# dazchi/gym-uav-collision-avoidance

Hardware: NVIDIA B200
Metric: UAV env-steps/sec (higher is better)
Workload: dtype f64 velocity / f32 position+obs (as the reference)

## Files before the change

gym_uav_collision_avoidance_b200/csrc/uavca_kernels.cu:

```cuda
#include <atomic>
#include <cmath>
#include <cstdlib>

#include "uavca_host.h"
#include "uavca_multi.cuh"
#include "uavca_seq.cuh"
#include "uavca_cta.cuh"
#include "uavca_tma.cuh"

namespace uavca {


struct GlobalIO {
  const KernelArgs& a;
  const Lane& L;
  float* stage;
  __device__ __forceinline__ Uav load_uav() const { return uavca::load_uav(a.s, L); }
  __device__ __forceinline__ float2 load_action() const {
    return L.valid ? ld_stream(a.io.action + L.m) : make_float2(0.f, 0.f);
  }
  __device__ __forceinline__ int load_steps() const { return L.valid ? a.s.steps[L.env] : 0; }
  __device__ __forceinline__ void loads_done() const { cudaTriggerProgrammaticLaunchCompletion(); }
  __device__ __forceinline__ void store_reward_done(float r, bool done) const {
    if (L.valid) {
// ... 279 lines not shown
                      L.valid ? a.s.steps[L.env] : 0, (unsigned)L.m};
    cudaTriggerProgrammaticLaunchCompletion();
    const unsigned M = (unsigned)r.M;
    if constexpr (KIND == kRolloutPlainBlock) {
      const unsigned end = r.KM + (unsigned)L.m;
      if (L.valid) cp_async8(slot, r.action_block + io.off);
      do {
        cp_async_wait_all();
        io.act = L.valid ? lds_float2(slot) : make_float2(0.f, 0.f);
        const unsigned next = io.off + M;
        if (next < end && L.valid) cp_async8(slot ^ 256u, r.action_block + next);
        step_core<NT>(a, ws, L, io);
        io.off = next;
        slot ^= 256u;
      } while (io.off < end);
    } else {
      uint4 words = make_uint4(0u, 0u, 0u, 0u);
      for (int k = 0; k < r.K; ++k) {
        const unsigned long long t = r.step0 + (unsigned long long)k;
        if (k == 0 || (t & 1ull) == 0ull) words = action_words(r.seed_lo, r.seed_hi, env_global, L.i, t);
        io.act = map_action(action_from_words(words, t), UAVCA_ACTION_SCALED, a.c);
        step_core<NT>(a, ws, L, io);
        io.off += M;
      }
    }
    store_uav(a.s, L, io.cur, true);
    if (L.valid & (L.i == 0)) a.s.steps[L.env] = io.steps;
  } else {
    const bool block = r.action_block != nullptr;
    RolloutIO io{a, r, L, ws.stage, load_uav(a.s, L), make_float2(0.f, 0.f), L.valid ? a.s.steps[L.env] : 0, 0, 0};
    cudaTriggerProgrammaticLaunchCompletion();
    if (block && L.valid) cp_async8(slot, r.action_block + L.m);
    uint4 words = make_uint4(0u, 0u, 0u, 0u);
    for (int k = 0; k < r.K; ++k) {
      io.k = k;
      io.km = (long long)k * r.M;
      if (block) {
        cp_async_wait_all();
        io.act = L.valid ? lds_float2(slot + (k & 1) * 256) : make_float2(0.f, 0.f);
        if (k + 1 < r.K && L.valid) cp_async8(slot + ((k + 1) & 1) * 256, (r.action_block + (io.km + r.M)) + (unsigned)L.m);
      } else {
        const unsigned long long t = r.step0 + (unsigned long long)k;
        if (k == 0 || (t & 1ull) == 0ull) words = action_words(r.seed_lo, r.seed_hi, env_global, L.i, t);
        io.act = action_from_words(words, t);
        if (r.action_out != nullptr && L.valid) st_stream((r.action_out + io.km) + L.m, io.act);
      }
      step_core<NT>(a, ws, L, io);
    }
    store_uav(a.s, L, io.cur, true);
    if (L.valid & (L.i == 0)) a.s.steps[L.env] = io.steps;
  }
}

#ifndef UAVCA_ROLLOUT_MINB
#define UAVCA_ROLLOUT_MINB 8
#endif
template <int NT, int KIND>
__global__ void __launch_bounds__(kThreads, UAVCA_ROLLOUT_MINB) rollout_multi_kernel(const __grid_constant__ KernelArgs a,
                                                                                  const __grid_constant__ RolloutArgs r) {
  __shared__ __align__(16) float smem[kWarpsPerBlock * kScratchFloats];
  __shared__ __align__(512) float2 act_smem[kWarpsPerBlock * 64];
  const WarpScratch ws = warp_scratch(smem);
  const int warp_global = blockIdx.x * kWarpsPerBlock + (threadIdx.x >> 5);
  const int N = NT > 0 ? NT : a.N;
  const bool full = uavs_left(a.B, N, warp_global) >= (32 / N) * N;
  cudaGridDependencySynchronize();
  float2* const my_act = act_smem + (threadIdx.x >> 5) * 64;
  if (full) rollout_multi_body<NT, true, KIND>(a, r, ws, my_act, warp_global);
  else rollout_multi_body<NT, false, KIND>(a, r, ws, my_act, warp_global);
}

__global__ void __launch_bounds__(kThreads) sample_actions_kernel(const __grid_constant__ Consts c, float2* out, int B, int N,
                                                                  unsigned seed_lo, unsigned seed_hi, unsigned long long t) {
  const long long m = (long long)blockIdx.x * kThreads + threadIdx.x;
  if (m >= (long long)B * N) return;
  const long long env = m / N;
  const int i = (int)(m - env * N);
  out[m] = action_from_words(action_words(seed_lo, seed_hi, c.env_base + env, i, t), t);
}

constexpr int kPfStageBytes = 32 * (16 + 8 + 8 + 8 + 4 + 4);


struct PfStage {
  double2* vel;
  float2 *pos, *tgt, *act;
  float *init, *prev;
};
__device__ __forceinline__ PfStage pf_stage(unsigned char* base) {
  PfStage st;
  st.vel = reinterpret_cast<double2*>(base);
  st.pos = reinterpret_cast<float2*>(base + 32 * 16);
  st.tgt = st.pos + 32;
  st.act = st.tgt + 32;
  st.init = reinterpret_cast<float*>(st.act + 32);
  st.prev = st.init + 32;
  return st;
}

struct PfIO : GlobalIO {
  Uav pre;
  float2 act;
  int steps;
  __device__ __forceinline__ Uav load_uav() const { return pre; }
  __device__ __forceinline__ float2 load_action() const { return act; }
  __device__ __forceinline__ int load_steps() const { return steps; }
// ... 370 lines not shown
                                                                 float* o_mask, long long* o_idx) {
  const long long j = ((long long)blockIdx.x * kThreads + threadIdx.x) / kSampleLanes;
  const int l = threadIdx.x % kSampleLanes;
  if (j >= batch) return;
  const long long head = meta[0], size = meta[2];
  const unsigned long long ctr = draw + (unsigned long long)meta[3];
  const uint4 r = philox_indexed(kStreamSample, (unsigned long long)j, ctr, seed_lo, seed_hi);
  long long slot = 0;
  if (size > 0) {
    if (recency) {
      const double u = ((double)r.x + 0.5) * (1.0 / 4294967296.0);
      long long age = (long long)(sqrt(u) * (double)size);
      age = age >= size ? size - 1 : age;
      const long long oldest = size == cap ? head : 0;
      slot = oldest + age;
      slot -= slot >= cap ? cap : 0;
    } else {
      slot = (long long)(((unsigned long long)r.x * (unsigned long long)size) >> 32);
    }
  }
  for (int k = l; k < od; k += kSampleLanes) {
    o_obs[j * od + k] = r_obs[slot * od + k];
    o_nxt[j * od + k] = r_nxt[slot * od + k];
  }
  for (int k = l; k < ad; k += kSampleLanes) o_act[j * ad + k] = r_act[slot * ad + k];
  if (l == 0) {
    o_rew[j] = r_rew[slot];
    o_mask[j] = r_mask[slot];
    if (o_idx) o_idx[j] = slot;
  }
}


static inline int flat_grid(long long n) { return (int)((n + kThreads - 1) / kThreads); }

static inline int multi_grid(int B, int N) {
  const int epw = 32 / N;
  const long long warps = ((long long)B + epw - 1) / epw;
  return (int)((warps + kWarpsPerBlock - 1) / kWarpsPerBlock);
}

#define UAVCA_DISPATCH_N(N, CALL)            \
  switch (N) {                               \
    case 2: { constexpr int NT = 2; CALL; } break;   \
    case 4: { constexpr int NT = 4; CALL; } break;   \
    case 5: { constexpr int NT = 5; CALL; } break;   \
    case 8: { constexpr int NT = 8; CALL; } break;   \
    case 10: { constexpr int NT = 10; CALL; } break; \
    case 16: { constexpr int NT = 16; CALL; } break; \
    case 32: { constexpr int NT = 32; CALL; } break; \
    default: { constexpr int NT = 0; CALL; } break;  \
  }

template <int NT>
static cudaError_t launch_step_multi_n(const KernelArgs& a, int grid, cudaStream_t st) {
  cudaLaunchConfig_t cfg{};
  cfg.gridDim = dim3(grid);
  cfg.blockDim = dim3(kThreads);
  cfg.dynamicSmemBytes = 0;
  cfg.stream = st;
  cudaLaunchAttribute attr[1];
  attr[0].id = cudaLaunchAttributeProgrammaticStreamSerialization;
  attr[0].val.programmaticStreamSerializationAllowed = 1;
  cfg.attrs = attr;
  cfg.numAttrs = 1;
  return cudaLaunchKernelEx(&cfg, step_multi_kernel<NT>, a);
}


template <typename Kernel>
static cudaError_t launch_pdl(Kernel kernel, int grid, int threads, size_t smem, cudaStream_t st, const KernelArgs& a,
                              int num_tiles) {
  cudaLaunchConfig_t cfg{};
  cfg.gridDim = dim3(grid);
  cfg.blockDim = dim3(threads);
  cfg.dynamicSmemBytes = smem;
  cfg.stream = st;
  cudaLaunchAttribute attr[1];
  attr[0].id = cudaLaunchAttributeProgrammaticStreamSerialization;
  attr[0].val.programmaticStreamSerializationAllowed = 1;
  cfg.attrs = attr;
  cfg.numAttrs = 1;
  return cudaLaunchKernelEx(&cfg, kernel, a, num_tiles);
}

template <int NT, bool FINAL>
static cudaError_t launch_step_tma_n(const KernelArgs& a, int num_tiles, cudaStream_t st) {
  using G = TmaGeom<NT, FINAL>;
  constexpr int kMaxDev = 64;
  static std::atomic<int> slots[kMaxDev];
  int dev = 0;
  cudaError_t e = cudaGetDevice(&dev);
  if (e != cudaSuccess) return e;
  if (dev < 0 || dev >= kMaxDev) return cudaErrorInvalidDevice;
  auto kernel = step_multi_tma_kernel<NT, FINAL>;
  if (slots[dev] == 0) {
    e = cudaFuncSetAttribute(kernel, cudaFuncAttributeMaxDynamicSharedMemorySize, G::SMEM_BYTES);
    if (e != cudaSuccess) return e;
    int per_sm = 0, sms = 0;
    e = cudaOccupancyMaxActiveBlocksPerMultiprocessor(&per_sm, kernel, G::THREADS, G::SMEM_BYTES);
    if (e != cudaSuccess) return e;
    e = cudaDeviceGetAttribute(&sms, cudaDevAttrMultiProcessorCount, dev);
    if (e != cudaSuccess) return e;
    if (per_sm < 1) return cudaErrorLaunchOutOfResources;
    slots[dev] = per_sm * sms;
  }
// ... 173 lines not shown
  cfg.gridDim = dim3(grid);
  cfg.blockDim = dim3(kThreads);
  cfg.dynamicSmemBytes = 0;
  cfg.stream = st;
  cudaLaunchAttribute attr[1];
  attr[0].id = cudaLaunchAttributeProgrammaticStreamSerialization;
  attr[0].val.programmaticStreamSerializationAllowed = 1;
  cfg.attrs = attr;
  cfg.numAttrs = 1;
  return cudaLaunchKernelEx(&cfg, step_multi_ring_kernel<NT>, a, g);
}

cudaError_t launch_step_multi_ring(const KernelArgs& a, const RingSink& g, cudaStream_t st) {
  if (a.B <= 0) return cudaSuccess;
  if (wants_seq(a)) return cudaErrorNotSupported;
  cudaError_t e = cudaSuccess;
  UAVCA_DISPATCH_N(a.N, (e = launch_step_multi_ring_n<NT>(a, g, multi_grid(a.B, a.N), st)));
  if (e != cudaSuccess) return e;
  return cudaGetLastError();
}

template <typename Kernel>
static cudaError_t launch_pdl2(Kernel kernel, int grid, cudaStream_t st, const KernelArgs& a, const RolloutArgs& r) {
  cudaLaunchConfig_t cfg{};
  cfg.gridDim = dim3(grid);
  cfg.blockDim = dim3(kThreads);
  cfg.dynamicSmemBytes = 0;
  cfg.stream = st;
  cudaLaunchAttribute attr[1];
  attr[0].id = cudaLaunchAttributeProgrammaticStreamSerialization;
  attr[0].val.programmaticStreamSerializationAllowed = 1;
  cfg.attrs = attr;
  cfg.numAttrs = 1;
  return cudaLaunchKernelEx(&cfg, kernel, a, r);
}

cudaError_t launch_rollout_multi(const KernelArgs& a, const RolloutArgs& r, cudaStream_t st) {
  if (a.B <= 0 || r.K <= 0) return cudaSuccess;
  cudaError_t e = cudaSuccess;
  static const bool cta_ok = [] { const char* v = getenv("UAVCA_ROLLOUT_CTA"); return !(v && v[0] == '0'); }();
  if (cta_ok && cta_packs(a.N, true)) {
    const int envs_per_cta = kThreads / a.N;
    e = launch_pdl2(rollout_multi_cta_kernel, (a.B + envs_per_cta - 1) / envs_per_cta, st, a, r);
    return e != cudaSuccess ? e : cudaGetLastError();
  }
  const int grid = multi_grid(a.B, a.N);
  const bool block = r.action_block != nullptr;
  const bool plain = a.io.final_obs == nullptr && a.io.reset_mask == nullptr && !a.c.track_scores &&
                     (block ? a.io.action_mode == UAVCA_ACTION_CARTESIAN
                            : a.io.action_mode == UAVCA_ACTION_SCALED && r.action_out == nullptr) &&
                     (long long)r.K * r.M * UAVCA_OBS_DIM_MULTI < (1ll << 31);
  RolloutArgs rp = r;
  rp.KM = plain ? (unsigned)(r.K * r.M) : 0u;
  if (block && plain) {
    UAVCA_DISPATCH_N(a.N, (e = launch_pdl2(rollout_multi_kernel<NT, kRolloutPlainBlock>, grid, st, a, rp)));
  } else if (plain) {
    UAVCA_DISPATCH_N(a.N, (e = launch_pdl2(rollout_multi_kernel<NT, kRolloutPlainPhilox>, grid, st, a, rp)));
  } else {
    UAVCA_DISPATCH_N(a.N, (e = launch_pdl2(rollout_multi_kernel<NT, kRolloutGeneral>, grid, st, a, r)));
  }
  return e != cudaSuccess ? e : cudaGetLastError();
}

cudaError_t launch_rollout_single(const KernelArgs& a, const RolloutArgs& r, cudaStream_t st) {
  if (a.B <= 0 || r.K <= 0) return cudaSuccess;
  const cudaError_t e = launch_pdl2(rollout_single_kernel, flat_grid(a.B), st, a, r);
  return e != cudaSuccess ? e : cudaGetLastError();
}

cudaError_t launch_sample_actions(const Consts& c, float* out, int B, int N, unsigned long long seed, unsigned long long t,
                                  cudaStream_t st) {
  if (B <= 0) return cudaSuccess;
  sample_actions_kernel<<<flat_grid((long long)B * N), kThreads, 0, st>>>(c, reinterpret_cast<float2*>(out), B, N,
                                                                          (unsigned)(seed & 0xffffffffull),
                                                                          (unsigned)(seed >> 32), t);
  return cudaGetLastError();
}

cudaError_t launch_reset_multi(const KernelArgs& a, const uint8_t* mask, cudaStream_t st) {
  if (a.B <= 0) return cudaSuccess;
  if (wants_seq(a)) {
    if (a.c.circular) reset_multi_seq_kernel<double><<<flat_grid(a.B), kThreads, 0, st>>>(a, mask);
    else reset_multi_seq_kernel<float><<<flat_grid(a.B), kThreads, 0, st>>>(a, mask);
    return cudaGetLastError();
  }
  const int grid = multi_grid(a.B, a.N);
  UAVCA_DISPATCH_N(a.N, (reset_multi_kernel<NT><<<grid, kThreads, 0, st>>>(a, mask)));
  return cudaGetLastError();
}

cudaError_t launch_observe_multi(const KernelArgs& a, cudaStream_t st) {
  if (a.B <= 0) return cudaSuccess;
  if (wants_seq(a)) {
    if (a.c.circular) observe_multi_seq_kernel<double><<<flat_grid(a.B), kThreads, 0, st>>>(a);
    else observe_multi_seq_kernel<float><<<flat_grid(a.B), kThreads, 0, st>>>(a);
    return cudaGetLastError();
  }
  const int grid = multi_grid(a.B, a.N);
  UAVCA_DISPATCH_N(a.N, (observe_multi_kernel<NT><<<grid, kThreads, 0, st>>>(a)));
  return cudaGetLastError();
}

cudaError_t launch_step_single(const KernelArgs& a, cudaStream_t st) {
  if (a.B <= 0) return cudaSuccess;
  step_single_kernel<<<flat_grid(a.B), kThreads, 0, st>>>(a);
  return cudaGetLastError();
// ... 67 lines not shown
```

gym_uav_collision_avoidance_b200/csrc/uavca_multi.cuh:

```cuda
#pragma once

#include "uavca_device.cuh"

namespace uavca {

struct Lane {
  int N;
  int lanes_used;
  int lane;
  int i;
  int base;
  int ring;
  unsigned envmask;
  int env;
  int m;
  int warp_m0;
  int valid_lanes;
  bool valid;
};

__device__ __forceinline__ int uavs_left(int B, int N, int warp_global) { return (B - warp_global * (32 / N)) * N; }

template <int NT, bool FULL = false>
__device__ __forceinline__ Lane make_lane(int B, int Nrt, int warp_global) {
// ... 25 lines not shown
  return make_lane<NT, false>(B, Nrt, blockIdx.x * kWarpsPerBlock + (threadIdx.x >> 5));
}

struct Uav {
  float px, py, tx, ty, init, prev;
  double vx, vy;
  unsigned flags;
};

__device__ __forceinline__ Uav load_uav(const StateView& s, const Lane& L) {
  Uav u;
  if (L.valid) {
    float2 p = ld_stream(s.pos + L.m);
    double2 v = ld_stream(s.vel + L.m);
    float2 t = ld_stream(s.tgt + L.m);
    u.init = ld_stream(s.init + L.m);
    u.prev = ld_stream(s.prev + L.m);
    u.flags = ld_stream(s.flags + L.m);
    u.px = p.x; u.py = p.y; u.vx = v.x; u.vy = v.y; u.tx = t.x; u.ty = t.y;
  } else {
    u.px = u.py = u.ty = 0.f; u.tx = 8.f; u.init = u.prev = 8.f; u.vx = 1.0; u.vy = 0.0; u.flags = 0u;
  }
  return u;
}

__device__ __forceinline__ void store_uav(const StateView& s, const Lane& L, const Uav& u, bool with_target) {
  if (!L.valid) return;
  st_stream(s.pos + L.m, make_float2(u.px, u.py));
  st_stream(s.vel + L.m, make_double2(u.vx, u.vy));
  st_stream(s.prev + L.m, u.prev);
  st_stream(s.flags + L.m, (uint8_t)u.flags);
  if (with_target) {
    st_stream(s.tgt + L.m, make_float2(u.tx, u.ty));
    st_stream(s.init + L.m, u.init);
  }
}

struct WarpScratch {
  float4* pairs;
  float4* cand;
  float* th;
  float* stage;
  __device__ __forceinline__ float4* ring() const { return pairs; }
  __device__ __forceinline__ float* ring_th() const { return reinterpret_cast<float*>(pairs) + 256; }
};
constexpr int kMixedMaxN = 10;
template <int NT>
struct SweepKind {
  static constexpr bool kMixed = NT > 0 && NT <= kMixedMaxN;
};
constexpr int kRingFloats = 48 * 4 + 32 * 4 + 32;
constexpr int kScratchFloats = kRingFloats + 32 * 10;

__device__ __forceinline__ WarpScratch warp_scratch(float* block_smem) {
  float* w = block_smem + (threadIdx.x >> 5) * kScratchFloats;
  return WarpScratch{reinterpret_cast<float4*>(w), reinterpret_cast<float4*>(w + 192), w + 320, w + kRingFloats};
}

__device__ __forceinline__ void publish(const WarpScratch& ws, const Lane& L, float nx, float ny, float ox, float oy, float th_u) {
  if (L.valid) {
    float* ring = reinterpret_cast<float*>(ws.pairs + L.ring);
    const int s0 = L.i, s1 = L.i + L.N;
    const int a0 = ((s0 >> 1) << 2) + (s0 & 1), a1 = ((s1 >> 1) << 2) + (s1 & 1);
    ring[a0] = nx; ring[a0 + 2] = ny;
    ring[a1] = nx; ring[a1 + 2] = ny;
    ws.cand[L.lane] = make_float4(nx, ny, ox, oy);
    ws.th[L.lane] = th_u;
  }
  __syncwarp();
}


constexpr int kInfBits = 0x7f800000;

static __device__ __noinline__ int nearest2_exact(const float4* cand, int i, int N, float px, float py) {
  const float inf = __int_as_float(kInfBits);
  float s1 = inf, s2 = inf;
  int j1 = 0, j2 = 0;
  for (int k = 1; k < N; ++k) {
    int j = i + k;
    j -= j >= N ? N : 0;
    const float4 q = cand[j];
    const float s = sq32(__fsub_rn(q.x, px), __fsub_rn(q.y, py));
    const bool p1 = s < s1, p2 = s < s2;
    j2 = p1 ? j1 : (p2 ? k : j2);
    s2 = p1 ? s1 : (p2 ? s : s2);
    j1 = p1 ? k : j1;
    s1 = p1 ? s : s1;
  }
  return j1 | (j2 << 8);
}

static __device__ __noinline__ float nearest_mixed_exact(const float4* cand, int i, int N, float px, float py) {
  float smin = __int_as_float(kInfBits);
  for (int j = 0; j < N; ++j) {
    if (j == i) continue;
    const float4 q = cand[j];
    const float s = j < i ? sq32(__fsub_rn(q.x, px), __fsub_rn(q.y, py)) : sq32(__fsub_rn(q.z, px), __fsub_rn(q.w, py));
    smin = fminf(smin, s);
  }
  return smin;
}

template <int NT>
__device__ __forceinline__ void pair_scan(const Consts& c, const WarpScratch& ws, const Lane& L, float px, float py,
                                          int& k1, int& k2, int& t3_out) {
  const int N = NT > 0 ? NT : L.N;
  const int k0 = L.i & 1;
  const float4* row = ws.pairs + L.ring + ((L.i + 1) >> 1);
  const float2 npx = make_float2(-px, -px), npy = make_float2(-py, -py), zero = make_float2(0.f, 0.f);
  auto dist2 = [&](int p) {
    const float4 q = row[p];
    const float2 dx = __fadd2_rn(make_float2(q.x, q.y), npx), dy = __fadd2_rn(make_float2(q.z, q.w), npy);
    return __fadd2_rn(__ffma2_rn(dx, dx, zero), __ffma2_rn(dy, dy, zero));
  };
  const int mask = c.key_mask;
  auto key = [&](float sq, int e) {
    int kk = (__float_as_int(sq) & mask) | e;
    if (e >= N) return kInfBits + 5 * 32;
    if (e == 0) kk = k0 ? kk : kInfBits + 3 * 32;
    if (e == N - 1) kk = k0 ? kInfBits + 4 * 32 : kk;
    return kk;
// ... 35 lines not shown
  float2 a, b, c;
};
__device__ __forceinline__ ObsTail obs_tail(const Consts& c, float dx1, float dy1, float dx2, float dy2, float s1, float s2,
                                            float h1, float h2, bool have1, bool have2, float th_u) {
  const float2 b = fast_atan2_pair(dy1, dx1, dy2, dx2);
  const float2 nth = make_float2(-th_u, -th_u);
  const float2 v1 = wrap_units2(__ffma2_rn(b, make_float2(c.inv_pi, c.inv_pi), nth));
  const float2 v2 = wrap_units2(__fadd2_rn(make_float2(h1, h2), nth));
  const float2 d = __fmul2_rn(make_float2(sqrt_approx(s1), sqrt_approx(s2)), make_float2(c.inv_dsense, c.inv_dsense));
  ObsTail o;
  o.a.x = have1 ? d.x : 1.0f;
  o.a.y = have1 ? v1.x : 1.0f;
  o.b.x = have1 ? v2.x : 0.0f;
  o.b.y = have2 ? d.y : 1.0f;
  o.c.x = have2 ? v1.y : 1.0f;
  o.c.y = have2 ? v2.y : 0.0f;
  return o;
}

template <int NT, bool WANT_A>
__device__ __forceinline__ ObsTail neighbours(const Consts& c, const WarpScratch& ws, const Lane& L, float px, float py,
                                              float th_u, int k1, int k2, int t3, float& smin) {
  const int N = NT > 0 ? NT : L.N;
  int j1 = L.i + k1, j2 = L.i + k2;
  const bool w1 = j1 >= N, w2 = j2 >= N;
  j1 -= w1 ? N : 0;
  j2 -= w2 ? N : 0;
  const float4 q1 = ws.cand[L.base + j1], q2 = ws.cand[L.base + j2];
  const float h1 = ws.th[L.base + j1], h2 = ws.th[L.base + j2];
  const float dx1 = __fsub_rn(q1.x, px), dy1 = __fsub_rn(q1.y, py), dx2 = __fsub_rn(q2.x, px), dy2 = __fsub_rn(q2.y, py);
  const float s1 = sq32(dx1, dy1), s2 = sq32(dx2, dy2);
  if (WANT_A) {
    const float inf = __int_as_float(kInfBits);
    float a1 = w1 ? s1 : sq32(__fsub_rn(q1.z, px), __fsub_rn(q1.w, py));
    float a2 = w2 ? s2 : sq32(__fsub_rn(q2.z, px), __fsub_rn(q2.w, py));
    a1 = k1 != 0 ? a1 : inf;
    a2 = k2 != 0 ? a2 : inf;
    smin = fminf(a1, a2);
    if (t3 <= c.near_key) smin = nearest_mixed_exact(ws.cand + L.base, L.i, N, px, py);
  }
  const bool have1 = (k1 != 0) & (s1 < c.s_dsense_lt);
  const bool have2 = have1 & (k2 != 0) & (s2 < c.s_dsense_lt);
  return obs_tail(c, dx1, dy1, dx2, dy2, s1, s2, h1, h2, have1, have2, th_u);
}

__device__ __forceinline__ void publish_mixed(const WarpScratch& ws, const Lane& L, float nx, float ny, float ox, float oy, float th_u) {
  if (L.valid) {
    const int slot = 2 * L.base + L.i;
    ws.ring()[slot] = make_float4(ox, nx, oy, ny);
    ws.ring()[slot + L.N] = make_float4(nx, nx, ny, ny);
    ws.ring_th()[slot] = th_u;
    ws.ring_th()[slot + L.N] = th_u;
  }
  __syncwarp();
}

static __device__ __noinline__ int nearest2_exact_ring(const float4* row, float px, float py, int N) {
  const float inf = __int_as_float(kInfBits);
  float s1 = inf, s2 = inf;
  int j1 = 0, j2 = 0;
  for (int k = 1; k < N; ++k) {
    const float4 q = row[k];
    const float s = sq32(__fsub_rn(q.y, px), __fsub_rn(q.w, py));
    const bool p1 = s < s1, p2 = s < s2;
    j2 = p1 ? j1 : (p2 ? k : j2);
    s2 = p1 ? s1 : (p2 ? s : s2);
    j1 = p1 ? k : j1;
    s1 = p1 ? s : s1;
  }
  return j1 | (j2 << 8);
}

template <int NT>
__device__ __forceinline__ void pair_scan_mixed(const Consts& c, const WarpScratch& ws, const Lane& L, float px, float py,
                                                float& smin, int& k1, int& k2) {
  constexpr int N = NT;
  const float4* row = ws.ring() + 2 * L.base + L.i;
  const float2 npx = make_float2(-px, -px), npy = make_float2(-py, -py), zero = make_float2(0.f, 0.f);
  auto dist2 = [&](int k) {
    const float4 q = row[k];
    const float2 dx = __fadd2_rn(make_float2(q.x, q.y), npx), dy = __fadd2_rn(make_float2(q.z, q.w), npy);
    return __fadd2_rn(__ffma2_rn(dx, dx, zero), __ffma2_rn(dy, dy, zero));
  };
  const int mask = c.key_mask;
  auto key = [mask](float sq, int k) { return (__float_as_int(sq) & mask) | k; };
  smin = __int_as_float(kInfBits);
  int t1 = kInfBits, t2 = kInfBits + 32, t3 = kInfBits + 64;
  int k = 1;
#pragma unroll
  for (; k + 1 < N; k += 2) {
    const float2 s0 = dist2(k), s1 = dist2(k + 1);
    smin = fminf(smin, fminf(s0.x, s1.x));
    const int ka = key(s0.y, k), kb = key(s1.y, k + 1);
    const int a = min(ka, kb), b = max(ka, kb);
    const int m1a = max(t1, a), m2a = max(t2, a), m1b = max(t1, b);
    t3 = __vimin3_s32(t3, m2a, m1b);
    t2 = __vimin3_s32(t2, m1a, b);
    t1 = min(t1, a);
  }
  if (k < N) {
    const float2 s0 = dist2(k);
    smin = fminf(smin, s0.x);
    const int a = key(s0.y, k);
    t3 = min(t3, max(t2, a));
    t2 = min(t2, max(t1, a));
    t1 = min(t1, a);
  }
  k1 = t1 & 31;
  k2 = t2 & 31;
  if (((unsigned)(t1 ^ t2) < 32u) | ((unsigned)(t2 ^ t3) < 32u)) {
    const int e = nearest2_exact_ring(row, px, py, N);
    k1 = e & 0xff;
    k2 = e >> 8;
  }
}

__device__ __forceinline__ ObsTail neighbours_mixed(const Consts& c, const WarpScratch& ws, const Lane& L, float px, float py,
                                                    float th_u, int k1, int k2) {
  const int slot = 2 * L.base + L.i;
  const float4 q1 = ws.ring()[slot + k1], q2 = ws.ring()[slot + k2];
  const float h1 = ws.ring_th()[slot + k1], h2 = ws.ring_th()[slot + k2];
  const float2 dx = __fadd2_rn(make_float2(q1.y, q2.y), make_float2(-px, -px)), dy = __fadd2_rn(make_float2(q1.w, q2.w), make_float2(-py, -py));
  const float2 zero = make_float2(0.f, 0.f), s = __fadd2_rn(__ffma2_rn(dx, dx, zero), __ffma2_rn(dy, dy, zero));
  const bool have1 = (k1 != 0) & (s.x < c.s_dsense_lt);
  const bool have2 = have1 & (k2 != 0) & (s.y < c.s_dsense_lt);
  return obs_tail(c, dx.x, dy.x, dx.y, dy.y, s.x, s.y, h1, h2, have1, have2, th_u);
}

template <int NT>
__device__ __forceinline__ ObsTail scan_neighbours(const Consts& c, const WarpScratch& ws, const Lane& L, float nx, float ny,
                                                   float ox, float oy, float th_u, float& smin) {
  int k1, k2;
  if (SweepKind<NT>::kMixed) {
    publish_mixed(ws, L, nx, ny, ox, oy, th_u);
    pair_scan_mixed<NT>(c, ws, L, nx, ny, smin, k1, k2);
    return neighbours_mixed(c, ws, L, nx, ny, th_u, k1, k2);
  }
  int t3;
  publish(ws, L, nx, ny, ox, oy, th_u);
  pair_scan<NT>(c, ws, L, nx, ny, k1, k2, t3);
  return neighbours<NT, true>(c, ws, L, nx, ny, th_u, k1, k2, t3, smin);
}

struct Own {
  float th_u, dth_u, dist, ssq;
  double vsq;
};
__device__ __forceinline__ Own own_features(const Consts& c, float px, float py, float tx, float ty, double vx, double vy) {
  Own w;
  const float2 td = __fadd2_rn(make_float2(tx, ty), make_float2(-px, -py));
  const float tdx = td.x, tdy = td.y;
  const float2 tsq = __ffma2_rn(td, td, make_float2(0.f, 0.f));
  w.ssq = __fadd_rn(tsq.x, tsq.y);
  w.dist = __fsqrt_rn(w.ssq);
  w.vsq = sq64(vx, vy);
  const float fvx = (float)vx, fvy = (float)vy;
  const bool vzero = (vx == 0.0) & (vy == 0.0);
  const float hx = vzero ? 1.0f : fvx;
  const float cr = fmaf(hx, tdy, -(fvy * tdx));
  const float dt = fmaf(hx, tdx, fvy * tdy);
  const float2 ang = fast_atan2_pair(fvy, fvx, cr, dt);
  w.th_u = ang.x * c.inv_pi;
  w.dth_u = ang.y * c.inv_pi;
  if ((!vzero & (fabsf(fvx) + fabsf(fvy) < 1e-30f)) | (w.ssq == 0.0f)) {
    const float2 s = angles_slow((double)tdx, (double)tdy, vx, vy);
    w.th_u = s.x; w.dth_u = s.y;
  }
  return w;
}

__device__ __forceinline__ void obs_own(const Consts& c, const Own& w, double vsq, float2& o01, float2& o23) {
  o01 = make_float2(sqrt_approx((float)vsq) * c.inv_vm2_f, w.th_u);
  o23 = make_float2(w.dist * c.inv_diag, w.dth_u);
}

struct ObsRow {
  float2 o01, o23;
  ObsTail n;
};
template <int NT>
__device__ __forceinline__ ObsRow observe_state(const Consts& c, const WarpScratch& ws, const Lane& L, const Uav& u) {
  const Own w = own_features(c, u.px, u.py, u.tx, u.ty, u.vx, u.vy);
  __syncwarp();
  ObsRow r;
  obs_own(c, w, w.vsq, r.o01, r.o23);
  float unused;
  r.n = scan_neighbours<NT>(c, ws, L, u.px, u.py, u.px, u.py, w.th_u, unused);
  return r;
}

__device__ __forceinline__ void stage_own(float* stage, int lane, float2 o01, float2 o23) {
  float2* row = reinterpret_cast<float2*>(stage) + lane * 5;
  row[0] = o01; row[1] = o23;
}
// ... 130 lines not shown
    const bool env_conflict = ((bal >> L.base) & L.envmask) != 0u;
    if (active) {
      if (env_conflict && att + 1u < kMaxResetAttempts) {
        if (L.i == cur) {
          ++attempt;
          tg = draw_pair(c, env_global, episode, kStreamTgt, L.i, attempt, c.lox, c.hix, c.loy, c.hiy);
        }
      } else {
        ++cur;
      }
    }
  }
  if (do_reset) {
    u.px = cand.x; u.py = cand.y; u.tx = tg.x; u.ty = tg.y;
    u.vx = 0.0; u.vy = 0.0; u.flags = 0u;
    u.init = n32(__fsub_rn(u.tx, u.px), __fsub_rn(u.ty, u.py));
    u.prev = u.init;
  }
}


__device__ __forceinline__ float env_sum(float v, const Lane& L) {
#pragma unroll
  for (int off = 1; off < 32; off <<= 1) {
    const float o = __shfl_down_sync(kFull, v, off);
    v += (L.i + off < L.N) ? o : 0.0f;
  }
  return v;
}

__device__ __forceinline__ void fold_scores(const StateView& s, int env) {
  const double2 sc = s.score[env];
  atomicAdd(reinterpret_cast<double*>(s.stats + 4), sc.x);
  atomicAdd(reinterpret_cast<double*>(s.stats + 5), sc.y);
  s.score[env] = make_double2(0.0, 0.0);
}

static __device__ __forceinline__ double2 finish_velocity(double vx, double vy, double vsq) {
  const double nv = sqrt(vsq);
  double fx = __dmul_rn(__ddiv_rn(vx, nv), 0.001), fy = __dmul_rn(__ddiv_rn(vy, nv), 0.001);
  if ((fx != fx) | (fy != fy)) { fx = 0.0; fy = 0.0; }
  return make_double2(fx, fy);
}

template <class IO, class = void>
struct io_action64 { static constexpr bool value = false; };
template <class IO>
struct io_action64<IO, decltype((void)IO::kAction64)> { static constexpr bool value = IO::kAction64; };
template <class IO, class = void>
struct io_plain { static constexpr bool value = false; };
template <class IO>
struct io_plain<IO, decltype((void)IO::kPlain)> { static constexpr bool value = IO::kPlain; };

template <int NT, class IO>
__device__ __forceinline__ void step_core(const KernelArgs& a, const WarpScratch& ws, const Lane& L, IO& io) {
  const Consts& c = a.c;
  constexpr bool kF64 = io_action64<IO>::value;
  constexpr bool kPlain = io_plain<IO>::value;

  Uav u = io.load_uav();
  float2 act = make_float2(0.f, 0.f);
  double2 act64 = make_double2(0.0, 0.0);
  if constexpr (kF64) act64 = io.load_action64();
  else act = io.load_action();
  const int steps_new = io.load_steps() + 1;
  io.loads_done();
  if constexpr (!kF64 && !kPlain) {
    if (a.io.action_mode != UAVCA_ACTION_CARTESIAN) act = map_action(act, a.io.action_mode, c);
  }

  const bool parked = (u.flags & UAVCA_FLAG_PARKED) != 0u;
  const float ox = u.px, oy = u.py;

  {
    double vx = u.vx, vy = u.vy;
    float px = u.px, py = u.py;
    if constexpr (kF64) integrate(act64.x, act64.y, vx, vy, px, py, c);
    else integrate((double)act.x, (double)act.y, vx, vy, px, py, c);
    if (!parked) { u.vx = vx; u.vy = vy; u.px = px; u.py = py; }
  }
  const Own w = own_features(c, u.px, u.py, u.tx, u.ty, u.vx, u.vy);
  const float dist = parked ? 0.f : w.dist;
  const float prev_d = parked ? 0.f : u.prev;

  float r;
  {
    const float inv_init = rcp_approx(u.init);
    const float m = fminf(c.vm2_f * inv_init, 1.0f);
    r = fmaf(50.0f * c.inv_vm2_f, __fsub_rn(prev_d, dist), -0.01f * m);
    const float q = dist * inv_init * (1.0f / 1.5f);
    r *= (r > 0.0f) ? (1.0f - q) : (1.0f + q);
    r = fmaf(-0.01f * 3.14159274101257324f, fabsf(w.dth_u), r);
  }

  float smin;
  const ObsTail tail = scan_neighbours<NT>(c, ws, L, u.px, u.py, ox, oy, w.th_u, smin);

  const bool collision = smin <= c.s_coll_le;
  r = collision ? -2.0f : r;
  const bool hard = (smin <= c.s_hard_le) & ((u.flags & (UAVCA_FLAG_PARKED | UAVCA_FLAG_COLLIDED)) == 0u) & L.valid;
  if (hard) u.flags |= UAVCA_FLAG_COLLIDED;

  const bool inside = (u.px >= c.lox_f) & (u.px <= c.hix_f) & (u.py >= c.loy_f) & (u.py <= c.hiy_f);
  const bool reached = (parked ? true : (w.ssq < c.s_reach_lt)) & !collision & (w.vsq < c.reach_speed_sq);
  const bool newly_reached = reached & !parked & L.valid;
  const bool done = (reached | (!inside & (a.io.evaluate == 0))) & L.valid;
  double vsq_obs = w.vsq;
  if (reached) {
    u.flags |= UAVCA_FLAG_PARKED;
    const double2 fv = finish_velocity(u.vx, u.vy, w.vsq);
    u.vx = fv.x; u.vy = fv.y;
    r += 10.0f;
    vsq_obs = sq64(u.vx, u.vy);
  }
  u.prev = dist;

  {
    float2 o01, o23;
    obs_own(c, w, vsq_obs, o01, o23);
    io.put_own(o01, o23);
    io.put_neighbours(tail);
  }
  io.store_reward_done(r, done);

  const unsigned done_env = (__ballot_sync(kFull, done) >> L.base) & L.envmask;
  const bool rs = (((done_env & c.rs_any_mask) != 0u) | (((done_env ^ L.envmask) | c.rs_all_off) == 0u) |
                   (steps_new >= c.steps_limit)) & L.valid;
  const bool leader = L.valid & (L.i == 0);
  if (leader) io.store_reset(rs);
  if (!kPlain && c.track_scores) {
    const float live = env_sum((done | !L.valid) ? 0.0f : r, L);
    if (leader) {
      double2 sc = a.s.score[L.env];
      sc.x += (double)r;
      sc.y += (double)live;
      a.s.score[L.env] = sc;
    }
  }
  const bool bad = (!(fabsf(r) <= 3.4e38f) | !(fabsf(u.px) + fabsf(u.py) <= 3.4e38f)) & L.valid;

  if (!__any_sync(kFull, rs | newly_reached | hard | bad)) {
    io.store_steps(steps_new, leader);
    io.commit_obs();
    if (io.wants_final()) io.commit_final();
    io.store_state(u);
    return;
  }

  const unsigned ev_reach = __ballot_sync(kFull, newly_reached), ev_coll = __ballot_sync(kFull, hard);
  const int reach_inc = __popc((ev_reach >> L.base) & L.envmask), coll_inc = __popc((ev_coll >> L.base) & L.envmask);
  {
    const unsigned ev_bad = __ballot_sync(kFull, bad);
    if (ev_bad != 0u && L.lane == 0) atomicAdd(a.s.stats + 6, (unsigned long long)__popc(ev_bad));
  }
  if (io.wants_final()) io.commit_final();
  if (!__any_sync(kFull, rs)) {
    io.store_steps(steps_new, leader);
    if (leader) {
      if (reach_inc) a.s.reach[L.env] += reach_inc;
      if (coll_inc) a.s.coll[L.env] += coll_inc;
    }
    io.commit_obs();
    io.store_state(u);
    return;
  }
  unsigned episode = 0;
  if (leader) episode = a.s.episode[L.env];
  episode = __shfl_sync(kFull, episode, L.base);
  if (leader) {
    if (rs) {
      if (episode > 0u) {
        atomicAdd(a.s.stats + 0, 1ull);
        atomicAdd(a.s.stats + 1, (unsigned long long)(a.s.reach[L.env] + reach_inc));
        atomicAdd(a.s.stats + 2, (unsigned long long)(a.s.coll[L.env] + coll_inc));
        atomicAdd(a.s.stats + 3, (unsigned long long)steps_new);
        if (c.track_scores) fold_scores(a.s, L.env);
      }
      a.s.reach[L.env] = 0; a.s.coll[L.env] = 0;
      a.s.episode[L.env] = episode + 1u;
    } else {
      if (reach_inc) a.s.reach[L.env] += reach_inc;
      if (coll_inc) a.s.coll[L.env] += coll_inc;
    }
  }
  io.store_steps(rs ? 0 : steps_new, leader);
  Uav nu = u;
  reset_multi(a, L, rs, episode, nu);
  const ObsRow no = observe_state<NT>(c, ws, L, nu);
  if (rs) {
    u = nu;
    io.put_own(no.o01, no.o23);
    io.put_neighbours(no.n);
  }
  io.commit_obs();
  io.store_state(u);
  if (rs) io.store_target(u);
}

}
```

Before: 56.30 billion.

## Process two warps' worth of environments per warp in plain rollout

Adds a paired rollout kernel in which each warp steps two warp-groups of environments, interleaving their movement, neighbour publish, sweep and settle phases. The two groups share one warp sync and one any-vote check for the rare path, and observation rows are staged in shared memory and flushed as coalesced float4 streams. The aim is more independent work per warp to hide latency, along with amortised syncs and action prefetches. In exchange, register and shared-memory use grow (minimum blocks per SM drops to 4), which lowers occupancy, and the rare path runs serially for both groups.

```diff
diff --git a/gym_uav_collision_avoidance_b200/csrc/uavca_kernels.cu b/gym_uav_collision_avoidance_b200/csrc/uavca_kernels.cu
--- a/gym_uav_collision_avoidance_b200/csrc/uavca_kernels.cu
+++ b/gym_uav_collision_avoidance_b200/csrc/uavca_kernels.cu
@@ -355,6 +355,113 @@
   }
 }
 
+struct PairRolloutIO : PlainRolloutIO {
+  __device__ __forceinline__ void put_own(float2 o01, float2 o23) const {
+    if (L.valid) stage_own(stage, L.lane, o01, o23);
+  }
+  __device__ __forceinline__ void put_neighbours(const ObsTail& n) const {
+    if (L.valid) stage_neighbours(stage, L.lane, n);
+  }
+  __device__ __forceinline__ void commit_obs() const {}
+};
+
+template <int NT>
+__device__ __forceinline__ void flush_pair_rows(unsigned stage, float* g, int lane) {
+  constexpr int n4 = (32 / NT) * NT * 5;
+  float4* g4 = reinterpret_cast<float4*>(g);
+  __syncwarp();
+#pragma unroll
+  for (int r = 0; r < (n4 + 31) / 32; ++r) {
+    const int k = lane + 32 * r;
+    if (k < n4) st_stream(g4 + k, lds_float4(stage + k * 16));
+  }
+  __syncwarp();
+}
+
+template <int NT, int KIND>
+__device__ __forceinline__ void rollout_multi_pair_body(const KernelArgs& a, const RolloutArgs& r, const WarpScratch& wsA,
+                                                        const WarpScratch& wsB, unsigned stage, unsigned slot, int pair) {
+  constexpr int kUsed = (32 / NT) * NT;
+  const Lane LA = make_lane<NT, true>(a.B, a.N, 2 * pair), LB = make_lane<NT, true>(a.B, a.N, 2 * pair + 1);
+  const bool valid = LA.valid;
+  PairRolloutIO ioA{{a, LA, stage, load_uav(a.s, LA), make_float2(0.f, 0.f), valid ? a.s.steps[LA.env] : 0, (unsigned)LA.m}};
+  PairRolloutIO ioB{{a, LB, stage + kUsed * 40u, load_uav(a.s, LB), make_float2(0.f, 0.f), valid ? a.s.steps[LB.env] : 0,
+                     (unsigned)LB.m}};
+  cudaTriggerProgrammaticLaunchCompletion();
+  const unsigned M = (unsigned)r.M;
+  auto obs_run = [&] { return a.io.obs + (ioA.off - (unsigned)LA.lane) * (unsigned)UAVCA_OBS_DIM_MULTI; };
+  if constexpr (KIND == kRolloutPlainBlock) {
+    const unsigned end = r.KM + (unsigned)LA.m;
+    if (valid) {
+      cp_async8(slot, r.action_block + ioA.off);
+      cp_async8(slot + 512u, r.action_block + (ioA.off + kUsed));
+    }
+    do {
+      cp_async_wait_all();
+      ioA.act = valid ? lds_float2(slot) : make_float2(0.f, 0.f);
+      ioB.act = valid ? lds_float2(slot + 512u) : make_float2(0.f, 0.f);
+      const unsigned next = ioA.off + M;
+      if (next < end && valid) {
+        cp_async8(slot ^ 256u, r.action_block + next);
+        cp_async8((slot ^ 256u) + 512u, r.action_block + (next + kUsed));
+      }
+      ioB.off = ioA.off + kUsed;
+      step_pair<NT>(a, wsA, wsB, LA, LB, ioA, ioB);
+      flush_pair_rows<NT>(stage, obs_run(), LA.lane);
+      ioA.off = next;
+      slot ^= 256u;
+    } while (ioA.off < end);
+  } else {
+    const long long envA = a.c.env_base + LA.env, envB = a.c.env_base + LB.env;
+    uint4 wa = make_uint4(0u, 0u, 0u, 0u), wb = wa;
+    for (int k = 0; k < r.K; ++k) {
+      const unsigned long long t = r.step0 + (unsigned long long)k;
+      if (k == 0 || (t & 1ull) == 0ull) {
+        wa = action_words(r.seed_lo, r.seed_hi, envA, LA.i, t);
+        wb = action_words(r.seed_lo, r.seed_hi, envB, LB.i, t);
+      }
+      ioA.act = map_action(action_from_words(wa, t), UAVCA_ACTION_SCALED, a.c);
+      ioB.act = map_action(action_from_words(wb, t), UAVCA_ACTION_SCALED, a.c);
+      ioB.off = ioA.off + kUsed;
+      step_pair<NT>(a, wsA, wsB, LA, LB, ioA, ioB);
+      flush_pair_rows<NT>(stage, obs_run(), LA.lane);
+      ioA.off += M;
+    }
+  }
+  store_uav(a.s, LA, ioA.cur, true);
+  store_uav(a.s, LB, ioB.cur, true);
+  if (valid & (LA.i == 0)) {
+    a.s.steps[LA.env] = ioA.steps;
+    a.s.steps[LB.env] = ioB.steps;
+  }
+}
+
+#ifndef UAVCA_ROLLOUT_PAIR_MINB
+#define UAVCA_ROLLOUT_PAIR_MINB 4
+#endif
+constexpr int kPairWarpFloats = 2 * kRingFloats + 64 * 10;
+template <int NT, int KIND>
+__global__ void __launch_bounds__(kThreads, UAVCA_ROLLOUT_PAIR_MINB)
+    rollout_multi_pair_kernel(const __grid_constant__ KernelArgs a, const __grid_constant__ RolloutArgs r) {
+  __shared__ __align__(16) float smem[kWarpsPerBlock * kPairWarpFloats];
+  __shared__ __align__(512) float2 act_smem[kWarpsPerBlock * 128];
+  float* const w = smem + (threadIdx.x >> 5) * kPairWarpFloats;
+  float* const stage = w + 2 * kRingFloats;
+  const WarpScratch wsA = scratch_at(w, stage), wsB = scratch_at(w + kRingFloats, stage);
+  float2* const my_act = act_smem + (threadIdx.x >> 5) * 128;
+  const int pair = blockIdx.x * kWarpsPerBlock + (threadIdx.x >> 5);
+  constexpr int kUsed = (32 / NT) * NT;
+  const int left = uavs_left(a.B, NT, 2 * pair);
+  cudaGridDependencySynchronize();
+  if (left >= 2 * kUsed) {
+    rollout_multi_pair_body<NT, KIND>(a, r, wsA, wsB, (unsigned)__cvta_generic_to_shared(stage),
+                                      (unsigned)__cvta_generic_to_shared(my_act + (threadIdx.x & 31)), pair);
+  } else if (left > 0) {
+    rollout_multi_body<NT, false, KIND>(a, r, wsA, my_act, 2 * pair);
+    if (left > kUsed) rollout_multi_body<NT, false, KIND>(a, r, wsA, my_act, 2 * pair + 1);
+  }
+}
+
 #ifndef UAVCA_ROLLOUT_MINB
 #define UAVCA_ROLLOUT_MINB 8
 #endif
@@ -831,6 +938,18 @@
     default: { constexpr int NT = 0; CALL; } break;  \
   }
 
+#define UAVCA_DISPATCH_PAIR_N(N, CALL)                   \
+  switch (N) {                                           \
+    case 2: { constexpr int NT = 2; CALL; } break;       \
+    case 4: { constexpr int NT = 4; CALL; } break;       \
+    case 5: { constexpr int NT = 5; CALL; } break;       \
+    case 8: { constexpr int NT = 8; CALL; } break;       \
+    case 10: { constexpr int NT = 10; CALL; } break;     \
+    case 16: { constexpr int NT = 16; CALL; } break;     \
+    case 32: { constexpr int NT = 32; CALL; } break;     \
+    default: break;                                      \
+  }
+
 template <int NT>
 static cudaError_t launch_step_multi_n(const KernelArgs& a, int grid, cudaStream_t st) {
   cudaLaunchConfig_t cfg{};
@@ -1110,6 +1229,18 @@
                      (long long)r.K * r.M * UAVCA_OBS_DIM_MULTI < (1ll << 31);
   RolloutArgs rp = r;
   rp.KM = plain ? (unsigned)(r.K * r.M) : 0u;
+  if (plain) {
+    bool paired = false;
+    const int epw = 32 / a.N;
+    const long long pairs = (((long long)a.B + epw - 1) / epw + 1) / 2;
+    const int pgrid = (int)((pairs + kWarpsPerBlock - 1) / kWarpsPerBlock);
+    if (block) {
+      UAVCA_DISPATCH_PAIR_N(a.N, (paired = true, e = launch_pdl2(rollout_multi_pair_kernel<NT, kRolloutPlainBlock>, pgrid, st, a, rp)));
+    } else {
+      UAVCA_DISPATCH_PAIR_N(a.N, (paired = true, e = launch_pdl2(rollout_multi_pair_kernel<NT, kRolloutPlainPhilox>, pgrid, st, a, rp)));
+    }
+    if (paired) return e != cudaSuccess ? e : cudaGetLastError();
+  }
   if (block && plain) {
     UAVCA_DISPATCH_N(a.N, (e = launch_pdl2(rollout_multi_kernel<NT, kRolloutPlainBlock>, grid, st, a, rp)));
   } else if (plain) {
diff --git a/gym_uav_collision_avoidance_b200/csrc/uavca_multi.cuh b/gym_uav_collision_avoidance_b200/csrc/uavca_multi.cuh
--- a/gym_uav_collision_avoidance_b200/csrc/uavca_multi.cuh
+++ b/gym_uav_collision_avoidance_b200/csrc/uavca_multi.cuh
@@ -101,9 +101,12 @@
 constexpr int kRingFloats = 48 * 4 + 32 * 4 + 32;
 constexpr int kScratchFloats = kRingFloats + 32 * 10;
 
+__device__ __forceinline__ WarpScratch scratch_at(float* w, float* stage) {
+  return WarpScratch{reinterpret_cast<float4*>(w), reinterpret_cast<float4*>(w + 192), w + 320, stage};
+}
 __device__ __forceinline__ WarpScratch warp_scratch(float* block_smem) {
   float* w = block_smem + (threadIdx.x >> 5) * kScratchFloats;
-  return WarpScratch{reinterpret_cast<float4*>(w), reinterpret_cast<float4*>(w + 192), w + 320, w + kRingFloats};
+  return scratch_at(w, w + kRingFloats);
 }
 
 __device__ __forceinline__ void publish(const WarpScratch& ws, const Lane& L, float nx, float ny, float ox, float oy, float th_u) {
@@ -116,7 +119,6 @@
     ws.cand[L.lane] = make_float4(nx, ny, ox, oy);
     ws.th[L.lane] = th_u;
   }
-  __syncwarp();
 }
 
 
@@ -258,7 +260,6 @@
     ws.ring_th()[slot] = th_u;
     ws.ring_th()[slot + L.N] = th_u;
   }
-  __syncwarp();
 }
 
 static __device__ __noinline__ int nearest2_exact_ring(const float4* row, float px, float py, int N) {
@@ -334,18 +335,29 @@
 }
 
 template <int NT>
+__device__ __forceinline__ void publish_neighbours(const WarpScratch& ws, const Lane& L, float nx, float ny, float ox, float oy,
+                                                   float th_u) {
+  if (SweepKind<NT>::kMixed) publish_mixed(ws, L, nx, ny, ox, oy, th_u);
+  else publish(ws, L, nx, ny, ox, oy, th_u);
+}
+template <int NT>
+__device__ __forceinline__ ObsTail sweep_neighbours(const Consts& c, const WarpScratch& ws, const Lane& L, float nx, float ny,
+                                                    float th_u, float& smin) {
+  int k1, k2;
+  if (SweepKind<NT>::kMixed) {
+    pair_scan_mixed<NT>(c, ws, L, nx, ny, smin, k1, k2);
+    return neighbours_mixed(c, ws, L, nx, ny, th_u, k1, k2);
+  }
+  int t3;
+  pair_scan<NT>(c, ws, L, nx, ny, k1, k2, t3);
+  return neighbours<NT, true>(c, ws, L, nx, ny, th_u, k1, k2, t3, smin);
+}
+template <int NT>
 __device__ __forceinline__ ObsTail scan_neighbours(const Consts& c, const WarpScratch& ws, const Lane& L, float nx, float ny,
                                                    float ox, float oy, float th_u, float& smin) {
-  int k1, k2;
-  if (SweepKind<NT>::kMixed) {
-    publish_mixed(ws, L, nx, ny, ox, oy, th_u);
-    pair_scan_mixed<NT>(c, ws, L, nx, ny, smin, k1, k2);
-    return neighbours_mixed(c, ws, L, nx, ny, th_u, k1, k2);
-  }
-  int t3;
-  publish(ws, L, nx, ny, ox, oy, th_u);
-  pair_scan<NT>(c, ws, L, nx, ny, k1, k2, t3);
-  return neighbours<NT, true>(c, ws, L, nx, ny, th_u, k1, k2, t3, smin);
+  publish_neighbours<NT>(ws, L, nx, ny, ox, oy, th_u);
+  __syncwarp();
+  return sweep_neighbours<NT>(c, ws, L, nx, ny, th_u, smin);
 }
 
 struct Own {
@@ -582,25 +594,36 @@
 template <class IO>
 struct io_plain<IO, decltype((void)IO::kPlain)> { static constexpr bool value = IO::kPlain; };
 
+struct StepVals {
+  Uav u;
+  Own w;
+  float r, dist, ox, oy;
+  int steps_new;
+  bool parked, done, rs, newly_reached, hard, bad, leader;
+};
+
 template <int NT, class IO>
-__device__ __forceinline__ void step_core(const KernelArgs& a, const WarpScratch& ws, const Lane& L, IO& io) {
+__device__ __forceinline__ StepVals step_move(const KernelArgs& a, const Lane& L, IO& io) {
   const Consts& c = a.c;
   constexpr bool kF64 = io_action64<IO>::value;
   constexpr bool kPlain = io_plain<IO>::value;
-
-  Uav u = io.load_uav();
+  StepVals s;
+  Uav& u = s.u;
+
+  u = io.load_uav();
   float2 act = make_float2(0.f, 0.f);
   double2 act64 = make_double2(0.0, 0.0);
   if constexpr (kF64) act64 = io.load_action64();
   else act = io.load_action();
-  const int steps_new = io.load_steps() + 1;
+  s.steps_new = io.load_steps() + 1;
   io.loads_done();
   if constexpr (!kF64 && !kPlain) {
     if (a.io.action_mode != UAVCA_ACTION_CARTESIAN) act = map_action(act, a.io.action_mode, c);
   }
 
   const bool parked = (u.flags & UAVCA_FLAG_PARKED) != 0u;
-  const float ox = u.px, oy = u.py;
+  s.parked = parked;
+  s.ox = u.px; s.oy = u.py;
 
   {
     double vx = u.vx, vy = u.vy;
@@ -609,22 +632,31 @@
     else integrate((double)act.x, (double)act.y, vx, vy, px, py, c);
     if (!parked) { u.vx = vx; u.vy = vy; u.px = px; u.py = py; }
   }
-  const Own w = own_features(c, u.px, u.py, u.tx, u.ty, u.vx, u.vy);
-  const float dist = parked ? 0.f : w.dist;
+  s.w = own_features(c, u.px, u.py, u.tx, u.ty, u.vx, u.vy);
+  const float dist = parked ? 0.f : s.w.dist;
   const float prev_d = parked ? 0.f : u.prev;
-
-  float r;
+  s.dist = dist;
+
   {
     const float inv_init = rcp_approx(u.init);
     const float m = fminf(c.vm2_f * inv_init, 1.0f);
-    r = fmaf(50.0f * c.inv_vm2_f, __fsub_rn(prev_d, dist), -0.01f * m);
+    float r = fmaf(50.0f * c.inv_vm2_f, __fsub_rn(prev_d, dist), -0.01f * m);
     const float q = dist * inv_init * (1.0f / 1.5f);
     r *= (r > 0.0f) ? (1.0f - q) : (1.0f + q);
-    r = fmaf(-0.01f * 3.14159274101257324f, fabsf(w.dth_u), r);
-  }
-
-  float smin;
-  const ObsTail tail = scan_neighbours<NT>(c, ws, L, u.px, u.py, ox, oy, w.th_u, smin);
+    s.r = fmaf(-0.01f * 3.14159274101257324f, fabsf(s.w.dth_u), r);
+  }
+  return s;
+}
+
+template <int NT, class IO>
+__device__ __forceinline__ void step_settle(const KernelArgs& a, const Lane& L, IO& io, StepVals& s, const ObsTail& tail,
+                                            float smin) {
+  const Consts& c = a.c;
+  constexpr bool kPlain = io_plain<IO>::value;
+  Uav& u = s.u;
+  const Own& w = s.w;
+  const bool parked = s.parked;
+  float r = s.r;
 
   const bool collision = smin <= c.s_coll_le;
   r = collision ? -2.0f : r;
@@ -643,7 +675,7 @@
     r += 10.0f;
     vsq_obs = sq64(u.vx, u.vy);
   }
-  u.prev = dist;
+  u.prev = s.dist;
 
   {
     float2 o01, o23;
@@ -655,7 +687,7 @@
 
   const unsigned done_env = (__ballot_sync(kFull, done) >> L.base) & L.envmask;
   const bool rs = (((done_env & c.rs_any_mask) != 0u) | (((done_env ^ L.envmask) | c.rs_all_off) == 0u) |
-                   (steps_new >= c.steps_limit)) & L.valid;
+                   (s.steps_new >= c.steps_limit)) & L.valid;
   const bool leader = L.valid & (L.i == 0);
   if (leader) io.store_reset(rs);
   if (!kPlain && c.track_scores) {
@@ -668,19 +700,30 @@
     }
   }
   const bool bad = (!(fabsf(r) <= 3.4e38f) | !(fabsf(u.px) + fabsf(u.py) <= 3.4e38f)) & L.valid;
-
-  if (!__any_sync(kFull, rs | newly_reached | hard | bad)) {
-    io.store_steps(steps_new, leader);
-    io.commit_obs();
-    if (io.wants_final()) io.commit_final();
-    io.store_state(u);
-    return;
-  }
-
-  const unsigned ev_reach = __ballot_sync(kFull, newly_reached), ev_coll = __ballot_sync(kFull, hard);
+  s.r = r;
+  s.done = done; s.rs = rs; s.newly_reached = newly_reached; s.hard = hard; s.bad = bad; s.leader = leader;
+}
+
+__device__ __forceinline__ bool step_is_rare(const StepVals& s) { return s.rs | s.newly_reached | s.hard | s.bad; }
+
+template <class IO>
+__device__ __forceinline__ void step_finish(IO& io, const StepVals& s) {
+  io.store_steps(s.steps_new, s.leader);
+  io.commit_obs();
+  if (io.wants_final()) io.commit_final();
+  io.store_state(s.u);
+}
+
+template <int NT, class IO>
+__device__ __forceinline__ void step_rare(const KernelArgs& a, const WarpScratch& ws, const Lane& L, IO& io, const StepVals& s) {
+  const Consts& c = a.c;
+  Uav u = s.u;
+  const bool rs = s.rs, leader = s.leader;
+  const int steps_new = s.steps_new;
+  const unsigned ev_reach = __ballot_sync(kFull, s.newly_reached), ev_coll = __ballot_sync(kFull, s.hard);
   const int reach_inc = __popc((ev_reach >> L.base) & L.envmask), coll_inc = __popc((ev_coll >> L.base) & L.envmask);
   {
-    const unsigned ev_bad = __ballot_sync(kFull, bad);
+    const unsigned ev_bad = __ballot_sync(kFull, s.bad);
     if (ev_bad != 0u && L.lane == 0) atomicAdd(a.s.stats + 6, (unsigned long long)__popc(ev_bad));
   }
   if (io.wants_final()) io.commit_final();
@@ -727,4 +770,39 @@
   if (rs) io.store_target(u);
 }
 
-}
+template <int NT, class IO>
+__device__ __forceinline__ void step_core(const KernelArgs& a, const WarpScratch& ws, const Lane& L, IO& io) {
+  StepVals s = step_move<NT>(a, L, io);
+  float smin;
+  const ObsTail tail = scan_neighbours<NT>(a.c, ws, L, s.u.px, s.u.py, s.ox, s.oy, s.w.th_u, smin);
+  step_settle<NT>(a, L, io, s, tail, smin);
+  if (!__any_sync(kFull, step_is_rare(s))) {
+    step_finish(io, s);
+    return;
+  }
+  step_rare<NT>(a, ws, L, io, s);
+}
+
+template <int NT, class IO>
+__device__ __forceinline__ void step_pair(const KernelArgs& a, const WarpScratch& wsA, const WarpScratch& wsB,
+                                          const Lane& LA, const Lane& LB, IO& ioA, IO& ioB) {
+  StepVals sa = step_move<NT>(a, LA, ioA);
+  StepVals sb = step_move<NT>(a, LB, ioB);
+  publish_neighbours<NT>(wsA, LA, sa.u.px, sa.u.py, sa.ox, sa.oy, sa.w.th_u);
+  publish_neighbours<NT>(wsB, LB, sb.u.px, sb.u.py, sb.ox, sb.oy, sb.w.th_u);
+  __syncwarp();
+  float smin_a, smin_b;
+  const ObsTail ta = sweep_neighbours<NT>(a.c, wsA, LA, sa.u.px, sa.u.py, sa.w.th_u, smin_a);
+  const ObsTail tb = sweep_neighbours<NT>(a.c, wsB, LB, sb.u.px, sb.u.py, sb.w.th_u, smin_b);
+  step_settle<NT>(a, LA, ioA, sa, ta, smin_a);
+  step_settle<NT>(a, LB, ioB, sb, tb, smin_b);
+  if (!__any_sync(kFull, step_is_rare(sa) | step_is_rare(sb))) {
+    step_finish(ioA, sa);
+    step_finish(ioB, sb);
+    return;
+  }
+  step_rare<NT>(a, wsA, LA, ioA, sa);
+  step_rare<NT>(a, wsB, LB, ioB, sb);
+}
+
+}
```

After: 52.26 billion, median of 6. 7.2% lower.
